# autowarefoundation/autoware_vision_pilot

Measured on AMD Instinct MI355X. Metric: frames/sec (SceneSeg+Scene3D 1280x720, one camera per GPU: preprocess + shared encoder + 2 decoder(s) + decode per frame); p50 per-frame latency beside it, higher is better.
Workload: dtype fp16x3 (hi+lo fp16 pairs on the fp16 MFMA pipe, fp32 accumulate; fp32-class: floats within 1e-3 of the fp32 oracle, 0 class flips outside that float tolerance -- tie flips only, counted per pass in profiles/r06_parity_sweep.tsv); 1 GPU; BASELINE.json metric configuration: SceneSeg+Scene3D on one 1280x720 camera per GPU, batch 1, shared EfficientNet-B0 encoder (vp_create_shared), fp16x3; precision=fp16x3, parity_mode=True, frames_in_flight_per_gpu=3, net_input=1x3x320x640, gather=False

## Files before the change

### autoware_vision_pilot_amd/csrc/engine_dispatch.cpp

```cpp
#include "engine_internal.hpp"

namespace vp {

bool Engine::plan_latency() const { return (precision_ & 32) != 0 || dev_option_is("VP_PLAN_TARGET", 'l'); }

bool plan_override(const std::string& name, int* tile, int* nsplit) {
  const char* e = dev_option("VP_PLAN_OVERRIDE");
  if (!e) return false;
  const std::string s(e);
  size_t pos = 0;
  while (pos < s.size()) {
    size_t end = s.find(';', pos);
    if (end == std::string::npos) end = s.size();
    const std::string item = s.substr(pos, end - pos);
    pos = end + 1;
    const size_t eq = item.rfind('=');
    if (eq == std::string::npos || eq == 0) continue;
    const std::string key = item.substr(0, eq), val = item.substr(eq + 1);
    if (name.size() < key.size() || name.compare(name.size() - key.size(), key.size(), key) != 0) continue;
    const size_t colon = val.find(':');
    *tile = std::atoi(val.substr(0, colon).c_str());
    *nsplit = colon == std::string::npos ? 0 : std::atoi(val.substr(colon + 1).c_str());
    return true;
  }
// ... 180 lines not shown
    if (fits && want8) halo = 8;
  }
  if ((halo == 3 || halo == 8) && q.split && q.tile < 0 && c->nsplit == 1 && q.cin_pad % 32 == 0 && !q.logits_out && !q.in2 && stride1 && plain &&
      dev_option_is("VP_X3_T16", '1') && M >= 12800)
    halo = 9;
  return halo;
}

}

ConvChoice choose_conv(const std::string& name, const ConvQuery& q) {
  const int cstride = std::max(1, q.stride);
  if (cstride > 1 && (q.ks != 3 || q.H % cstride || q.W % cstride)) throw std::invalid_argument("strided conv: 3x3 on even maps only: " + name);
  const int M = (q.H / cstride) * (q.W / cstride), ncols = round_up(q.cout, 32);
  int halo = -1, rule_nsplit = 0;
  if (q.ks == 3 && cstride == 1 && q.H >= 8 && q.W >= 16) {
    halo = base_halo_tile(q, ncols);
    halo = pipelined_tile(q, ncols, halo, &rule_nsplit);
    halo = map_tile(q, ncols, M, halo);
    if (halo == 12 && (!q.split || q.fp8_storage || !conv3x3_map2_shape_ok(q.H, q.W, q.cin_pad, round_up(ncols, 64))))
      throw std::invalid_argument("halo tile 12 (map kernel, 64-channel slabs): parity mode, maps that tile into 20x40 regions, >= 32 input channels: " + name);
    if (q.fp8_storage && q.tile < 0 && halo >= 0) halo = ncols <= 32 ? 4 : 3;
    if (halo == 11 && (q.fp8_storage || (!q.split && q.cin_pad % 32 != 0) || !conv3x3_map_shape_ok(q.H, q.W, q.cin_pad, round_up(ncols, 32))))
      throw std::invalid_argument("halo tile 11 (map kernel): maps that tile into 20x40 or 10x20 regions, >= 32 input channels (a multiple of 32 in the fp16 engines): " + name);
    if (halo >= 6 && halo <= 9 && !q.split && q.cin_pad % 64 != 0) throw std::invalid_argument("halo tiles 6 - 9 in the fp16 engines: input channels a multiple of 64: " + name);
  }
  ConvChoice c;
  if (halo >= 0) {
    const int forced = q.nsplit > 0 ? q.nsplit : rule_nsplit;
    c.bk = 32;
    c.CoutW = round_up(ncols, halo_tile_co(halo));
// ... 423 lines not shown
```

### autoware_vision_pilot_amd/csrc/kernels_conv3x3_x3.hip

```cpp
#include <algorithm>
#include <cstdlib>
#include <type_traits>

#include "conv_epilogue.hpp"
#include "lds_dma.hpp"

namespace vp {

template <int CO_TILE, int TH, int WCO, int WPX, bool HDB, int ACT, int ABL = 0, bool SPLITK = false, bool X1 = false>
__global__ __launch_bounds__(64 * WCO * WPX, (CO_TILE == 64 && TH == 8) ? 3 : 2) void conv3x3_x3_kernel(const ConvGemmParams p) {
  constexpr int NTH = 64 * WCO * WPX;
  constexpr int TW = 16, ROWB = 80, HWD = TW + 2, HPX = (TH + 2) * HWD, PX = TH * TW;
  constexpr int HALO_BYTES = HPX * ROWB, WROW = 64, W_BYTES = CO_TILE * WROW;
  constexpr int HCHUNKS = HPX * 4, HP = (HCHUNKS + NTH - 1) / NTH;
  constexpr int MT = CO_TILE / WCO / 32, NT = PX / WPX / 32;
  constexpr int NHB = HDB ? 2 : 1;
  constexpr int PL = 2;
  constexpr int HSTRIDE = HALO_BYTES;
  constexpr int LT = 0;
  constexpr int RING = HP > 3 ? HP : 3;
  static_assert(MT >= 1 && NT >= 1 && HP <= 6 && (HP <= 3 || !HDB), "tile shape");
  extern __shared__ __attribute__((aligned(16))) char smem[];
  char* const halo_base = smem;
  char* const w_base = smem + NHB * PL * HSTRIDE;
// ... 50 lines not shown
    const bool ok = hidx < HCHUNKS && (unsigned)gy < (unsigned)p.H && (unsigned)gx < (unsigned)p.W;
    h_goff[pc] = ok ? (gy * p.W + gx) * p.Cin + ch * 8 : -1;
    if constexpr ((ABL & 512) != 0) h_goff[pc] = ok ? ((gy >> 1) * (p.W >> 1) + (gx >> 1)) * p.Cin + ch * 8 : -1;
  }
  const size_t w_goff0 = (size_t)c_first * 9 * w_step + co0 * 32 + wave * 512 + lane * 8;

  f32x16_t acc[MT][NT];
#pragma unroll
  for (int i = 0; i < MT; ++i)
#pragma unroll
    for (int j = 0; j < NT; ++j)
#pragma unroll
      for (int r = 0; r < 16; ++r) acc[i][j][r] = 0.0f;

  h8_t fa[2][MT], fal[2][MT], fb[2][NT], fbl[2][NT];
  constexpr bool DIRECT_A = (ABL & 4096) != 0;
  h8_t ra[DIRECT_A ? 3 : 1][2][MT], ral[DIRECT_A ? 3 : 1][2][MT];
  const size_t w_a0 = (size_t)c_first * 9 * w_step + co0 * 32;
  u32x4 rh_hi[RING], rh_lo[RING];
#pragma unroll
  for (int r = 0; r < RING; ++r) rh_hi[r] = rh_lo[r] = zero4;
  const int s_last = KC * 9 - 1;

#define VP_DMA_W(BUF, SIDX)                                                                  \
  {                                                                                          \
    const int si_ = (SIDX) < s_last ? (SIDX) : s_last;                                       \
    const size_t base_ = (size_t)si_ * w_step + w_goff0;                                     \
    char* dst_ = w_base + (BUF) * PL * W_BYTES + wave * 1024;                                \
    _Pragma("unroll") for (int pc = 0; pc < WPIECES; ++pc) {                                 \
      VP_GLOBAL_LOAD_LDS16(p.w_hi + base_ + pc * NW * 512, dst_ + pc * NW * 1024);           \
      VP_GLOBAL_LOAD_LDS16(p.w_lo + base_ + pc * NW * 512, dst_ + W_BYTES + pc * NW * 1024); \
// ... 28 lines not shown
#define VP_READ_FRAGS(SET, WBUF, HBUF, TAPOFS)                                               \
  {                                                                                          \
    const char* wsrc_ = (WBUF) + (a_ofs0 ^ ((SET) * 32));                                    \
    if constexpr (!DIRECT_A) {                                                               \
    _Pragma("unroll") for (int i = 0; i < MT; ++i) {                                         \
      fa[SET][i] = *reinterpret_cast<const h8_t*>(wsrc_ + i * WCO * 32 * WROW);              \
      fal[SET][i] = *reinterpret_cast<const h8_t*>(wsrc_ + W_BYTES + i * WCO * 32 * WROW);   \
    }                                                                                        \
    }                                                                                        \
    _Pragma("unroll") for (int j = 0; j < NT; ++j) {                                         \
      fb[SET][j] = *reinterpret_cast<const h8_t*>((HBUF) + b_ofs0 + j * 2 * HWD * ROWB + (TAPOFS) + (SET) * 32); \
      fbl[SET][j] = *reinterpret_cast<const h8_t*>((HBUF) + HSTRIDE + b_ofs0 + j * 2 * HWD * ROWB + (TAPOFS) + (SET) * 32); \
    }                                                                                        \
  }
#define VP_MFMA(SET) VP_MFMA_RANGE(SET, 0, MT * NT)
#define VP_MFMA_RANGE(SET, Q0, Q1)                                                           \
  _Pragma("unroll") for (int q_ = (Q0); q_ < (Q1); ++q_) {                                   \
    const int i = q_ / NT, j = q_ % NT;                                                      \
    if constexpr ((ABL & 2) != 0) { acc[i][j][0] += (float)fa[SET][i][0] + (float)fal[SET][i][1] + (float)fb[SET][j][2] + (float)fbl[SET][j][3]; continue; } \
    if constexpr (DIRECT_A) {                                                                \
      acc[i][j] = __builtin_amdgcn_mfma_f32_32x32x16_f16(ral[aslot_][SET][i], fb[SET][j], acc[i][j], 0, 0, 0); \
      acc[i][j] = __builtin_amdgcn_mfma_f32_32x32x16_f16(ra[aslot_][SET][i], fbl[SET][j], acc[i][j], 0, 0, 0); \
      acc[i][j] = __builtin_amdgcn_mfma_f32_32x32x16_f16(ra[aslot_][SET][i], fb[SET][j], acc[i][j], 0, 0, 0);  \
      continue;                                                                              \
    }                                                                                        \
    if constexpr (X1) {                      \
      acc[i][j] = __builtin_amdgcn_mfma_f32_32x32x16_f16(fa[SET][i], fb[SET][j], acc[i][j], 0, 0, 0);   \
      acc[i][j] = __builtin_amdgcn_mfma_f32_32x32x16_f16(fal[SET][i], fbl[SET][j], acc[i][j], 0, 0, 0); \
      continue;                                                                              \
    }                                                                                        \
    acc[i][j] = __builtin_amdgcn_mfma_f32_32x32x16_f16(fal[SET][i], fb[SET][j], acc[i][j], 0, 0, 0); \
    acc[i][j] = __builtin_amdgcn_mfma_f32_32x32x16_f16(fa[SET][i], fbl[SET][j], acc[i][j], 0, 0, 0); \
    acc[i][j] = __builtin_amdgcn_mfma_f32_32x32x16_f16(fa[SET][i], fb[SET][j], acc[i][j], 0, 0, 0);  \
  }
#define VP_TAP(T)                                                                            \
  {                                                                                          \
    constexpr int tap_ofs_ = (((T) / 3) * HWD + ((T) % 3)) * ROWB;                           \
    constexpr int aslot_ = DIRECT_A ? (T) % 3 : 0;    \
    constexpr int tn_ = ((T) + 1) % 9;                                                       \
    constexpr int tap_next_ = ((tn_ / 3) * HWD + (tn_ % 3)) * ROWB;                          \
    const char* wcur_ = w_base + ((T) % 3) * PL * W_BYTES;                                   \
    const char* wnext_ = w_base + (((T) + 1) % 3) * PL * W_BYTES;                            \
    const char* hnext_ = ((T) == 8 && HDB) ? hbuf_other : hbuf;                              \
     \
     \
     \
     \
     \
     \
     \
     \
     \
     \
    if constexpr (HDB && (T) == 3 && !(ABL & 1) && !(ABL & 64)) {                            \
      if (next_chunk) { _Pragma("unroll") for (int pc = 0; pc < HP; ++pc) VP_STORE_H(pc, pc, hb ^ 1) } \
    }                                                                                        \
    if constexpr (DIRECT_A) {                                                                \
      if (next_chunk || (T) < 7) VP_LOAD_A(((T) + 2) % 3, c * 9 + (T) + 2)                   \
    } else if constexpr (!(ABL & 1) && !(ABL & 128)) {                                       \
      if (next_chunk || (T) < 7) VP_DMA_W(((T) + 2) % 3, c * 9 + (T) + 2)                     \
    }                                                                                        \
    __builtin_amdgcn_sched_barrier(0);                                                       \
    VP_MFMA_RANGE(0, 0, MT * NT / 2)                                                         \
    __builtin_amdgcn_sched_barrier(0);                                                       \
    if constexpr (!(ABL & 4)) VP_READ_FRAGS(1, wcur_, hbuf, tap_ofs_)                        \
    __builtin_amdgcn_sched_barrier(0);  \
    if constexpr (HDB && (T) == LT && !(ABL & 1) && !(ABL & 64)) {                           \
      _Pragma("unroll") for (int pc = 0; pc < HP; ++pc) VP_LOAD_H(pc, pc, next_chunk ? c + 1 : c) \
    }                                                                                        \
    if constexpr (!HDB && (T) < HP && !(ABL & 1) && !(ABL & 64)) {                           \
      if (next_chunk) VP_LOAD_H((T) % RING, (T) < HP ? (T) : 0, c + 1)                       \
    }                                                                                        \
    VP_MFMA_RANGE(0, MT * NT / 2, MT * NT)                                                   \
// ... 71 lines not shown
    const char* hbuf = halo_base + (HDB ? hb : 0) * PL * HSTRIDE;
    const char* hbuf_other = halo_base + (HDB ? (hb ^ 1) : 0) * PL * HSTRIDE;
    VP_TAP(0) VP_TAP(1) VP_TAP(2) VP_TAP(3) VP_TAP(4) VP_TAP(5) VP_TAP(6) VP_TAP(7) VP_TAP(8)
    hb ^= 1;
  }
  if constexpr ((ABL & 32) != 0) {
    if (blockIdx.x == 0 && tid == 0) {
      unsigned long long* dst = reinterpret_cast<unsigned long long*>(p.partial);
      dst[0] = __builtin_readcyclecounter() - probe_c0;
      dst[1] = __builtin_amdgcn_s_memrealtime() - probe_w0;
    }
  }
#undef VP_TAP
#undef VP_MFMA
#undef VP_MFMA_RANGE
#undef VP_READ_FRAGS
#undef VP_STORE_H
#undef VP_LOAD_H
#undef VP_LOAD_A
#undef VP_DMA_W

  constexpr int PITCH = CO_TILE * 2 + 16, STAGE_PLANE = PX * PITCH;
  static_assert(PL * STAGE_PLANE <= NHB * PL * HSTRIDE + 3 * PL * W_BYTES, "stage fits the main buffers");
  if constexpr ((ABL & 16) != 0) {
    if (p.H == -12345) {
#pragma unroll
      for (int i = 0; i < MT; ++i)
#pragma unroll
        for (int j = 0; j < NT; ++j)
#pragma unroll
          for (int r = 0; r < 16; ++r) p.out_f32[(i * NT + j) * 16 + r + tid * 64] = acc[i][j][r];
    }
    return;
  }
  if constexpr (SPLITK) {
    const PixPatch<TW> pixs{y0, x0, p.H, p.W};
    const int M = p.H * p.W;
#pragma unroll
// ... 53 lines not shown
    *reinterpret_cast<h8_t*>(p.out_hi + o) = *reinterpret_cast<const h8_t*>(smem + r * PITCH + c8 * 16);
    if constexpr (!X1) *reinterpret_cast<h8_t*>(p.out_lo + o) = *reinterpret_cast<const h8_t*>(smem + STAGE_PLANE + r * PITCH + c8 * 16);
  }
}

bool conv3x3_x3_supported(const ConvGemmParams& p, int shape) {
  const int co_tile = (shape == 8 || shape == 9) ? 64 : 128;
  const bool x1 = p.in_lo == nullptr;
  if (!(p.ks == 3 && p.stride <= 1 && p.in_hi && p.w_hi && p.w_lo && p.CoutW % co_tile == 0 && p.Cin % (x1 ? 64 : 32) == 0 && p.Cin2 == 0 && p.nsplit >= 1)) return false;
  const bool act_ok = x1 ? (p.act == ACT_GELU_F16 || p.act == ACT_NONE) : (p.act == ACT_GELU || p.act == ACT_NONE);
  const bool plain = p.out_hi && (x1 ? p.out_lo == nullptr : p.out_lo != nullptr) && p.store_mode == STORE_NHWC && p.res_mode == RES_NONE && p.post_act == ACT_NONE && act_ok;
  if (p.nsplit > 1) return p.partial != nullptr && p.nsplit <= p.Cin / (x1 ? 64 : 32);
  return plain;
}

template <int CO, int TH, int WPX, bool HDB, bool X1, int WCO = 2>
static hipError_t launch_x3_cfg(const ConvGemmParams& p, hipStream_t st) {
  constexpr int lds = (HDB ? 2 : 1) * 2 * ((TH + 2) * 18 * 80) + 6 * (CO * 64);
  static_assert(lds <= 160 * 1024, "LDS budget");
  constexpr int GELU = X1 ? ACT_GELU_F16 : ACT_GELU;
  const bool gelu = p.act == GELU, sk = p.nsplit > 1;
  auto k = sk ? conv3x3_x3_kernel<CO, TH, WCO, WPX, HDB, ACT_NONE, 0, true, X1>
              : (gelu ? conv3x3_x3_kernel<CO, TH, WCO, WPX, HDB, GELU, 0, false, X1> : conv3x3_x3_kernel<CO, TH, WCO, WPX, HDB, ACT_NONE, 0, false, X1>);
  static LdsAttrOnce attr_once[3];
  if (hipError_t e = set_max_dynamic_lds(attr_once[sk ? 2 : gelu], reinterpret_cast<const void*>(k), lds); e != hipSuccess) return e;
  dim3 grid(((p.H + TH - 1) / TH) * ((p.W + 15) / 16) * (p.CoutW / CO) * p.nsplit);
  hipLaunchKernelGGL(k, grid, dim3(64 * WCO * WPX), lds, st, p);
  hipError_t e = hipGetLastError();
  if (e != hipSuccess) return e;
  return sk ? launch_splitk_finish(p, st) : hipSuccess;
}

hipError_t launch_conv3x3_x3(const ConvGemmParams& p, int shape, hipStream_t st) {
  if (!conv3x3_x3_supported(p, shape)) return hipErrorInvalidValue;
  if (p.in_lo == nullptr) {
    if (shape == 6) return launch_x3_cfg<128, 16, 4, true, true>(p, st);
    if (shape == 7) return launch_x3_cfg<128, 8, 2, false, true>(p, st);
    if (shape == 8) return launch_x3_cfg<64, 8, 2, false, true>(p, st);
    if (shape == 9) return launch_x3_cfg<64, 16, 4, false, true, 1>(p, st);
    return hipErrorInvalidValue;
  }
  if (shape == 6) return launch_x3_cfg<128, 16, 4, true, false>(p, st);
  if (shape == 7) return launch_x3_cfg<128, 8, 2, false, false>(p, st);
  if (shape == 8) return launch_x3_cfg<64, 8, 2, false, false>(p, st);
  if (shape == 9) return launch_x3_cfg<64, 16, 4, false, false, 1>(p, st);
  return hipErrorInvalidValue;
}

}
```

### autoware_vision_pilot_amd/csrc/kernels_upconv.hip

```cpp
#include <algorithm>
#include <cstdlib>

#include "conv_epilogue.hpp"
#include "lds_dma.hpp"

namespace vp {

namespace {

struct PixPhase {
  int y0, x0, H, W, py, px;
  __device__ __forceinline__ int operator()(int q) const {
    int rowbit, c;
    lane_to_px16(q & 31, rowbit, c);
    const int y = y0 + 2 * (q >> 5) + rowbit, x = x0 + c;
    return (y < H && x < W) ? (2 * y + py) * (2 * W) + 2 * x + px : -1;
  }
};
struct PixRun {
  int kA, kE, W, py, px;
  __device__ __forceinline__ int operator()(int q) const {
    int rowbit, c;
    lane_to_px16(q & 31, rowbit, c);
    const int k = kA + (q >> 5) * 32 + 16 * rowbit + c;
    if (k >= kE) return -1;
    const int y = k / W, x = k - y * W;
    return (2 * y + py) * (2 * W) + 2 * x + px;
  }
};
constexpr int upconv_halo_bytes(int TH, bool CPT) { return (CPT && TH == 8) ? 192 * 80 : (TH + 2) * 18 * 80; }
constexpr int upconv_halo_capacity(int nth) { return 3 * nth / 4; }
__device__ __forceinline__ int bias_class(int m, int H2, int W2) {
  const int Y = m / W2, X = m - Y * W2;
  return (Y == 0 ? 0 : (Y == H2 - 1 ? 2 : 1)) * 3 + (X == 0 ? 0 : (X == W2 - 1 ? 2 : 1));
}

}

#define VP_WAIT_VMCNT_RT(N)                       \
  do {                                            \
    const int n_ = (N);                           \
    if (n_ >= 16) { VP_WAIT_VMCNT(16); }          \
    else if (n_ >= 14) { VP_WAIT_VMCNT(14); }     \
    else if (n_ >= 12) { VP_WAIT_VMCNT(12); }     \
    else if (n_ >= 10) { VP_WAIT_VMCNT(10); }     \
    else if (n_ >= 8) { VP_WAIT_VMCNT(8); }       \
    else if (n_ >= 6) { VP_WAIT_VMCNT(6); }       \
    else if (n_ >= 4) { VP_WAIT_VMCNT(4); }       \
    else if (n_ >= 2) { VP_WAIT_VMCNT(2); }       \
    else { VP_WAIT_VMCNT(0); }                    \
  } while (0)

template <int CO_TILE, int TH, int WCO, int WPX, bool HDB, int ACT, bool SPLITK, bool X1 = false, int ABL = 0, bool CPT = false>
__global__ __launch_bounds__(64 * WCO * WPX, 2) void upconv_x3_kernel(const UpconvParams p) {
  constexpr int NTH = 64 * WCO * WPX;
  constexpr int TW = 16, ROWB = 80, HWD = TW + 2, HPX = (TH + 2) * HWD, PX = TH * TW;
  constexpr int HALO_BYTES = upconv_halo_bytes(TH, CPT), WROW = 64, W_BYTES = CO_TILE * WROW;
  constexpr int HCHUNKS = HPX * 4, HP = (HCHUNKS + NTH - 1) / NTH;
  constexpr int MT = CO_TILE / WCO / 32, NT = PX / WPX / 32;
  constexpr int NHB = HDB ? 2 : 1;
  constexpr int PL = 2;
  constexpr int HSTRIDE = HALO_BYTES;
  static_assert(MT >= 1 && NT >= 1 && HP <= 3, "tile shape");
  extern __shared__ __attribute__((aligned(16))) char smem[];
  char* const halo_base = smem;
  char* const w_base = smem + NHB * PL * HSTRIDE;

  const int tid = threadIdx.x, lane = tid & 63, wave = tid >> 6;
// ... 91 lines not shown
    h_gs[pc] = ok ? (4 * gy * p.W + 2 * gx) * p.Cs + ch * 8 : -1;
  }
  const UpconvChunk dA = upconv_chunk(cA, py, px, CinV, CsV);
  const int S = (cB < n_chunks ? upconv_chunk(cB, py, px, CinV, CsV).step0 : upconv_steps(CinV, CsV)) - dA.step0;
  const size_t w_goff0 = ((size_t)phase * upconv_steps(CinV, CsV) + dA.step0) * w_step + co0 * 32 + wave * 512 + lane * 8;

  f32x16_t acc[MT][NT];
#pragma unroll
  for (int i = 0; i < MT; ++i)
#pragma unroll
    for (int j = 0; j < NT; ++j)
#pragma unroll
      for (int r = 0; r < 16; ++r) acc[i][j][r] = 0.0f;

  h8_t fa[2][MT], fal[2][MT], fb[2][NT], fbl[2][NT];
  u32x4 rh_hi[HP], rh_lo[HP];
#pragma unroll
  for (int r = 0; r < HP; ++r) rh_hi[r] = rh_lo[r] = zero4;

#define VP_DMA_W(WOFS, SIDX)                                                                 \
  if (!(ABL & 128) || (SIDX) < 2) {                                                          \
    const size_t base_ = (size_t)(SIDX) * w_step + w_goff0;                                  \
    char* dst_ = w_base + (WOFS) + wave * 1024;                                              \
    _Pragma("unroll") for (int pc = 0; pc < WPIECES; ++pc) {                                 \
      VP_GLOBAL_LOAD_LDS16(p.w_hi + base_ + pc * NW * 512, dst_ + pc * NW * 1024);           \
      VP_GLOBAL_LOAD_LDS16(p.w_lo + base_ + pc * NW * 512, dst_ + W_BYTES + pc * NW * 1024); \
    }                                                                                        \
  }
#define VP_LOAD_H(D)                                                                         \
  if (!(ABL & 1) || abl_prologue) {                                                          \
    const half_t* sh_ = (D).skip ? p.sk_hi : p.in_hi;                                        \
    const half_t* sl_ = (D).skip ? (VP_SK_DEAD1(D) ? p.sk_hi : sk_p1) : in_p1;               \
    const int add_ = (D).skip ? ((D).qy * 2 * p.W + (D).qx) * p.Cs + CHM * (D).ch0 : CHM * (D).ch0; \
    _Pragma("unroll") for (int pc = 0; pc < HP; ++pc) {                                      \
      const int g_ = (D).skip ? h_gs[pc] : h_gx[pc];                                         \
      const int o_ = (g_ >= 0 ? g_ + add_ : 0);                                              \
      rh_hi[pc] = *reinterpret_cast<const u32x4*>(sh_ + o_);                                 \
      rh_lo[pc] = *reinterpret_cast<const u32x4*>(sl_ + o_);                                 \
    }                                                                                        \
  }
#define VP_STORE_H(BUF, DEAD1)                                                               \
  if (!(ABL & 1) || abl_prologue)                                                            \
  _Pragma("unroll") for (int pc = 0; pc < HP; ++pc) {                                        \
    if (CPT ? h_ls[pc] >= 0 : tid + NTH * pc < HCHUNKS) {                                    \
      char* dst_ = halo_base + (BUF) * PL * HSTRIDE + (CPT ? h_ls[pc] : h_lds0 + pc * (NTH / 4) * ROWB); \
      *reinterpret_cast<u32x4*>(dst_) = h_gx[pc] >= 0 ? rh_hi[pc] : zero4;                   \
      *reinterpret_cast<u32x4*>(dst_ + HSTRIDE) = (h_gx[pc] >= 0 && !(DEAD1)) ? rh_lo[pc] : zero4; \
    }                                                                                        \
  }
#define VP_READ_FRAGS(SET, WPTR, HPTR, TAPOFS)                                               \
  {                                                                                          \
    const char* wsrc_ = (WPTR) + (a_ofs0 ^ ((SET) * 32));                                    \
    if (!CPT || nlj > 0)                                                                     \
    _Pragma("unroll") for (int i = 0; i < MT; ++i) {                                         \
      fa[SET][i] = *reinterpret_cast<const h8_t*>(wsrc_ + i * WCO * 32 * WROW);              \
      fal[SET][i] = *reinterpret_cast<const h8_t*>(wsrc_ + W_BYTES + i * WCO * 32 * WROW);   \
    }                                                                                        \
    if constexpr (CPT) {                                                                     \
      const char* hsrc_ = (HPTR) + (TAPOFS) + (SET) * 32;                                    \
      _Pragma("unroll") for (int j = 0; j < NT; ++j) {                                       \
        if (j >= nlj) continue;                                                              \
        fb[SET][j] = *reinterpret_cast<const h8_t*>(hsrc_ + b_ofs[j]);                       \
        fbl[SET][j] = *reinterpret_cast<const h8_t*>(hsrc_ + HSTRIDE + b_ofs[j]);            \
      }                                                                                      \
    } else {                                                                                 \
      const char* hsrc_ = (HPTR) + b_ofs0 + (TAPOFS) + (SET) * 32;                           \
      _Pragma("unroll") for (int j = 0; j < NT; ++j) {                                       \
        fb[SET][j] = *reinterpret_cast<const h8_t*>(hsrc_ + j * 2 * HWD * ROWB);             \
        fbl[SET][j] = *reinterpret_cast<const h8_t*>(hsrc_ + HSTRIDE + j * 2 * HWD * ROWB);  \
      }                                                                                      \
    }                                                                                        \
  }
#define VP_MFMA_RANGE(SET, Q0, Q1)                                                           \
  _Pragma("unroll") for (int q_ = (Q0); q_ < (Q1); ++q_) {                                   \
    const int i = q_ / NT, j = q_ % NT;                                                      \
    if constexpr (CPT) { if (j >= nlj) continue; }        \
    if constexpr ((ABL & 2) != 0) { acc[i][j][0] += (float)fa[SET][i][0] + (float)fal[SET][i][1] + (float)fb[SET][j][2] + (float)fbl[SET][j][3]; continue; } \
    if constexpr (X1) {                      \
      acc[i][j] = __builtin_amdgcn_mfma_f32_32x32x16_f16(fa[SET][i], fb[SET][j], acc[i][j], 0, 0, 0);   \
      acc[i][j] = __builtin_amdgcn_mfma_f32_32x32x16_f16(fal[SET][i], fbl[SET][j], acc[i][j], 0, 0, 0); \
      continue;                                                                              \
    }                                                                                        \
    acc[i][j] = __builtin_amdgcn_mfma_f32_32x32x16_f16(fal[SET][i], fb[SET][j], acc[i][j], 0, 0, 0); \
    acc[i][j] = __builtin_amdgcn_mfma_f32_32x32x16_f16(fa[SET][i], fbl[SET][j], acc[i][j], 0, 0, 0); \
    acc[i][j] = __builtin_amdgcn_mfma_f32_32x32x16_f16(fa[SET][i], fb[SET][j], acc[i][j], 0, 0, 0);  \
  }
#define VP_TAP_OFS(D, K) ((tpy + (D).a0 + ((D).nb == 2 ? ((K) >> 1) : (K))) * hrp + (tpx + (D).b0 + ((D).nb == 2 ? ((K) & 1) : 0)) * ROWB)

  bool abl_prologue = true;
  VP_LOAD_H(dA)
  VP_STORE_H(0, VP_SK_DEAD1(dA))
  VP_DMA_W(0, 0)
  if (S > 1) VP_DMA_W(PL * W_BYTES, 1)
  VP_WAIT_VMCNT(0);
  __syncthreads();
  UpconvChunk d = dA;
  UpconvChunk dn = dA;
  if (cA + 1 < cB) {
    dn = upconv_chunk(cA + 1, py, px, CinV, CsV);
    VP_LOAD_H(dn)
  }
  VP_READ_FRAGS(0, w_base, halo_base, VP_TAP_OFS(d, 0))
  abl_prologue = false;

  int c = cA, t = 0, s = 0, hb = 0;
  int w_cur = 0, w_nxt = PL * W_BYTES, w_fre = 2 * PL * W_BYTES;
#define VP_STEP(KIND, PREVLD)                                                                \
  {                                                                                          \
    const int tap_cur_ = VP_TAP_OFS(d, t);                                                   \
    const int tap_nxt_ = (KIND) == 0 ? VP_TAP_OFS(d, t + 1) : ((KIND) == 3 ? tap_cur_ : VP_TAP_OFS(dn, 0)); \
    const char* hbuf = halo_base + (HDB ? hb : 0) * PL * HSTRIDE;                            \
    const char* hbuf_next = (HDB && (KIND) != 0) ? halo_base + (hb ^ 1) * PL * HSTRIDE : hbuf; \
     \
     \
     \
    if constexpr (HDB && ((KIND) == 1 || (KIND) == 2)) { VP_STORE_H(hb ^ 1, VP_SK_DEAD1(dn)) }   \
     \
    if (s + 2 < S) VP_DMA_W(w_fre, s + 2)                                                    \
    __builtin_amdgcn_sched_barrier(0);                                                       \
    VP_MFMA_RANGE(0, 0, MT * NT / 2)                                                         \
    __builtin_amdgcn_sched_barrier(0);                                                       \
    VP_READ_FRAGS(1, w_base + w_cur, hbuf, tap_cur_)                                         \
    __builtin_amdgcn_sched_barrier(0);   \
    UpconvChunk dnn = dn;                                                                    \
    if constexpr (HDB && (KIND) == 1) {                                                      \
      dnn = upconv_chunk(c + 2, py, px, CinV, CsV);                                        \
      VP_LOAD_H(dnn)                                                                         \
    }                                                                                        \
    VP_MFMA_RANGE(0, MT * NT / 2, MT * NT)                                                   \
    __builtin_amdgcn_sched_barrier(0);                                                       \
     \
     \
    {                                                                                        \
      const int dma_n = s + 2 < S ? PL * WPIECES : 0;                                        \
      const int ld_prev = ((PREVLD) && t == 0) ? PL * HP : 0;                                \
      const int ld_this = (HDB && (KIND) == 1) ? PL * HP : 0;                                \
      VP_WAIT_VMCNT_RT(dma_n + ld_prev + ld_this);                                           \
    }                                                                                        \
     \
    VP_LDS_BARRIER();                                                                        \
    if constexpr (!HDB && ((KIND) == 1 || (KIND) == 2)) {                                    \
       \
       \
      VP_STORE_H(0, VP_SK_DEAD1(dn))                                                         \
      VP_LDS_BARRIER();                                                                      \
      if constexpr ((KIND) == 1) {                                                           \
        dnn = upconv_chunk(c + 2, py, px, CinV, CsV);                                      \
        VP_LOAD_H(dnn)                                                                       \
      }                                                                                      \
    }                                                                                        \
           \
    VP_READ_FRAGS(0, w_base + w_nxt, hbuf_next, tap_nxt_)                                    \
    __builtin_amdgcn_sched_barrier(0);                                                       \
    VP_MFMA_RANGE(1, 0, MT * NT)                                                             \
    __builtin_amdgcn_sched_barrier(0);                                                       \
                                    \
    {                                                                                        \
      const int w_old = w_cur;                                                               \
      w_cur = w_nxt;                                                                         \
      w_nxt = w_fre;                                                                         \
      w_fre = w_old;                                                                         \
    }                                                                                        \
    ++s;                                                                                     \
    if constexpr ((KIND) == 0) {                                                             \
      ++t;                                                                                   \
    } else {                                                                                 \
      ++c;                                                                                   \
      t = 0;                                                                                 \
      d = dn;                                                                                \
      dn = dnn;                                                                              \
      hb ^= 1;                                                                               \
    }                                                                                        \
  }
  while (c + 2 < cB) {
    while (t + 1 < d.nt) VP_STEP(0, true)
    VP_STEP(1, true)
  }
  if (c + 1 < cB) {
    while (t + 1 < d.nt) VP_STEP(0, true)
    VP_STEP(2, true)
  }
  while (t + 1 < d.nt) VP_STEP(0, false)
  VP_STEP(3, false)
#undef VP_STEP
#undef VP_SK_DEAD1
#undef VP_TAP_OFS
#undef VP_MFMA_RANGE
#undef VP_READ_FRAGS
#undef VP_STORE_H
#undef VP_LOAD_H
#undef VP_DMA_W

  const auto pix = [&] {
    if constexpr (CPT) return PixRun{kA, kE, p.W, py, px};
    else return PixPhase{y0, x0, p.H, p.W, py, px};
  }();
  if constexpr ((ABL & 16) != 0) {
    if (p.H == -12345) {
#pragma unroll
      for (int i = 0; i < MT; ++i)
#pragma unroll
        for (int j = 0; j < NT; ++j)
// ... 8 lines not shown
    for (int j = 0; j < NT; ++j) {
      const int m = pix((wpx * NT + j) * 32 + (lane & 31));
      if (m < 0) continue;
      float* row = p.partial + ((size_t)zsplit * M2 + m) * p.CoutW + co0 + 4 * (lane >> 5);
#pragma unroll
      for (int i = 0; i < MT; ++i)
#pragma unroll
        for (int g = 0; g < 4; ++g) {
          const f32x4_t v = {acc[i][j][4 * g + 0], acc[i][j][4 * g + 1], acc[i][j][4 * g + 2], acc[i][j][4 * g + 3]};
          *reinterpret_cast<f32x4_t*>(row + (i * WCO + wco) * 32 + 8 * g) = v;
        }
    }
    return;
  } else {
    constexpr int PITCH = CO_TILE * 2 + 16, STAGE_PLANE = PX * PITCH;
    static_assert(PL * STAGE_PLANE <= NHB * PL * HSTRIDE + 3 * PL * W_BYTES, "stage fits the main buffers");
    const float* const wsc = p.wscale + (size_t)phase * p.CoutW + co0;
    f32x4_t bb[NT][MT][4], sc[MT][4];
    int qpix[NT];
#pragma unroll
    for (int j = 0; j < NT; ++j) {
      qpix[j] = (wpx * NT + j) * 32 + (lane & 31);
      const int m = pix(qpix[j]);
      const float* const bsrc = p.bias + (size_t)(m >= 0 ? bias_class(m, 2 * p.H, 2 * p.W) : 4) * p.CoutW + co0;
#pragma unroll
      for (int i = 0; i < MT; ++i)
#pragma unroll
        for (int g = 0; g < 4; ++g) bb[j][i][g] = *reinterpret_cast<const f32x4_t*>(bsrc + (i * WCO + wco) * 32 + 4 * (lane >> 5) + 8 * g);
    }
#pragma unroll
    for (int i = 0; i < MT; ++i)
// ... 88 lines not shown
  const bool x1 = p.in_lo == nullptr;
  if (!(p.in_hi && p.w_hi && p.w_lo && p.bias && p.wscale && p.out_hi && (x1 ? p.out_lo == nullptr : p.out_lo != nullptr))) return false;
  if (p.H < 1 || p.W < 1 || p.Cin < (x1 ? 64 : 32) || p.Cin % (x1 ? 64 : 32) != 0 || p.Cs % 32 != 0 || p.Cs < 0) return false;
  if (p.Cs > 0 && !(p.sk_hi && (x1 ? p.sk_lo == nullptr : p.sk_lo != nullptr))) return false;
  if (p.CoutW % 128 != 0 || p.Ncols % 8 != 0 || p.Ncols > p.CoutW || p.Cstore < p.Ncols) return false;
  if (!(p.act == (x1 ? ACT_GELU_F16 : ACT_GELU) || p.act == ACT_NONE)) return false;
  if (p.nsplit < 1 || p.nsplit > (x1 ? upconv_chunks(p.Cin >> 1, ((p.Cs + 63) >> 6) << 5) : upconv_chunks(p.Cin, p.Cs))) return false;
  if (p.nsplit > 1 && !p.partial) return false;
  if ((long long)p.H * p.W * p.Cin >= (1ll << 31) || 4ll * p.H * p.W * std::max(p.Cs, 1) >= (1ll << 31) || 4ll * p.H * p.W * p.Cstore >= (1ll << 31)) return false;
  return true;
}

template <int TH, int WPX, bool HDB, bool X1, bool CPT = false>
static hipError_t launch_upconv_cfg(const UpconvParams& p, hipStream_t st) {
  constexpr int CO = 128;
  constexpr int lds = (HDB ? 2 : 1) * 2 * upconv_halo_bytes(TH, CPT) + 6 * (CO * 64);
  static_assert(lds <= (TH == 8 ? 80 : 160) * 1024, "LDS budget (the 4-wave shape: two workgroups per CU)");
  constexpr int GELU = X1 ? ACT_GELU_F16 : ACT_GELU;
  const bool gelu = p.act == GELU, sk = p.nsplit > 1;
  auto k = sk ? upconv_x3_kernel<CO, TH, 2, WPX, HDB, ACT_NONE, true, X1, 0, CPT>
              : (gelu ? upconv_x3_kernel<CO, TH, 2, WPX, HDB, GELU, false, X1, 0, CPT> : upconv_x3_kernel<CO, TH, 2, WPX, HDB, ACT_NONE, false, X1, 0, CPT>);
  static LdsAttrOnce attr_once[3];
  if (hipError_t e = set_max_dynamic_lds(attr_once[sk ? 2 : gelu], reinterpret_cast<const void*>(k), lds); e != hipSuccess) return e;
  const int n_px = CPT ? (p.H * p.W + TH * 16 - 1) / (TH * 16) : ((p.H + TH - 1) / TH) * ((p.W + 15) / 16);
  dim3 grid(n_px * 4 * (p.CoutW / CO) * p.nsplit);
  hipLaunchKernelGGL(k, grid, dim3(64 * 2 * WPX), lds, st, p);
  hipError_t e = hipGetLastError();
  if (e != hipSuccess || !sk) return e;
  const long long n = 4ll * p.H * p.W * (p.Ncols >> 3);
  hipLaunchKernelGGL(upconv_finish_kernel, dim3((unsigned)((n + 255) / 256)), dim3(256), 0, st, p);
  return hipGetLastError();
// ... 72 lines not shown
```

Before: 565.6 frames/s.

## Load conv weights directly into registers for the shape-7 x3 conv path

Shape 7 of the x3 3x3 conv now launches a direct-A variant whenever split-K is off. It uses 4 co-waves, one pixel wave and a double-buffered halo, and loads weight fragments from global memory straight into a 3-slot register ring instead of DMAing them into LDS. This drops the weight LDS buffers, shrinking LDS to the max of halo and staging so more workgroups fit per CU, and removes the LDS reads of weights. The upconv kernel gets the same direct-A machinery with a runtime-kind step loop, but its launcher still passes DA=false, so that path is inactive. The dispatcher also lets forced x3 tiles 106-109 apply to small maps. The risk is more register pressure and uncoalesced global weight reads per wave.

```diff
diff --git a/autoware_vision_pilot_amd/csrc/engine_dispatch.cpp b/autoware_vision_pilot_amd/csrc/engine_dispatch.cpp
--- a/autoware_vision_pilot_amd/csrc/engine_dispatch.cpp
+++ b/autoware_vision_pilot_amd/csrc/engine_dispatch.cpp
@@ -218,7 +218,8 @@
   if (cstride > 1 && (q.ks != 3 || q.H % cstride || q.W % cstride)) throw std::invalid_argument("strided conv: 3x3 on even maps only: " + name);
   const int M = (q.H / cstride) * (q.W / cstride), ncols = round_up(q.cout, 32);
   int halo = -1, rule_nsplit = 0;
-  if (q.ks == 3 && cstride == 1 && q.H >= 8 && q.W >= 16) {
+  const bool forced_x3 = q.tile >= 106 && q.tile <= 109;
+  if (q.ks == 3 && cstride == 1 && ((q.H >= 8 && q.W >= 16) || forced_x3)) {
     halo = base_halo_tile(q, ncols);
     halo = pipelined_tile(q, ncols, halo, &rule_nsplit);
     halo = map_tile(q, ncols, M, halo);
diff --git a/autoware_vision_pilot_amd/csrc/kernels_conv3x3_x3.hip b/autoware_vision_pilot_amd/csrc/kernels_conv3x3_x3.hip
--- a/autoware_vision_pilot_amd/csrc/kernels_conv3x3_x3.hip
+++ b/autoware_vision_pilot_amd/csrc/kernels_conv3x3_x3.hip
@@ -7,7 +7,12 @@
 
 namespace vp {
 
-template <int CO_TILE, int TH, int WCO, int WPX, bool HDB, int ACT, int ABL = 0, bool SPLITK = false, bool X1 = false>
+constexpr int x3_lds_bytes(int CO, int TH, bool HDB, bool DA) {
+  const int halo = (HDB ? 2 : 1) * 2 * ((TH + 2) * 18 * 80), stage = 2 * TH * 16 * (CO * 2 + 16);
+  return DA ? (halo > stage ? halo : stage) : halo + 6 * (CO * 64);
+}
+
+template <int CO_TILE, int TH, int WCO, int WPX, bool HDB, int ACT, int ABL = 0, bool SPLITK = false, bool X1 = false, bool DA = false>
 __global__ __launch_bounds__(64 * WCO * WPX, (CO_TILE == 64 && TH == 8) ? 3 : 2) void conv3x3_x3_kernel(const ConvGemmParams p) {
   constexpr int NTH = 64 * WCO * WPX;
   constexpr int TW = 16, ROWB = 80, HWD = TW + 2, HPX = (TH + 2) * HWD, PX = TH * TW;
@@ -88,7 +93,7 @@
       for (int r = 0; r < 16; ++r) acc[i][j][r] = 0.0f;
 
   h8_t fa[2][MT], fal[2][MT], fb[2][NT], fbl[2][NT];
-  constexpr bool DIRECT_A = (ABL & 4096) != 0;
+  constexpr bool DIRECT_A = DA;
   h8_t ra[DIRECT_A ? 3 : 1][2][MT], ral[DIRECT_A ? 3 : 1][2][MT];
   const size_t w_a0 = (size_t)c_first * 9 * w_step + co0 * 32;
   u32x4 rh_hi[RING], rh_lo[RING];
@@ -147,24 +152,20 @@
     }                                                                                        \
   }
 #define VP_MFMA(SET) VP_MFMA_RANGE(SET, 0, MT * NT)
+#define VP_A(SET, I) (DIRECT_A ? ra[aslot_][SET][I] : fa[SET][I])
+#define VP_AL(SET, I) (DIRECT_A ? ral[aslot_][SET][I] : fal[SET][I])
 #define VP_MFMA_RANGE(SET, Q0, Q1)                                                           \
   _Pragma("unroll") for (int q_ = (Q0); q_ < (Q1); ++q_) {                                   \
     const int i = q_ / NT, j = q_ % NT;                                                      \
-    if constexpr ((ABL & 2) != 0) { acc[i][j][0] += (float)fa[SET][i][0] + (float)fal[SET][i][1] + (float)fb[SET][j][2] + (float)fbl[SET][j][3]; continue; } \
-    if constexpr (DIRECT_A) {                                                                \
-      acc[i][j] = __builtin_amdgcn_mfma_f32_32x32x16_f16(ral[aslot_][SET][i], fb[SET][j], acc[i][j], 0, 0, 0); \
-      acc[i][j] = __builtin_amdgcn_mfma_f32_32x32x16_f16(ra[aslot_][SET][i], fbl[SET][j], acc[i][j], 0, 0, 0); \
-      acc[i][j] = __builtin_amdgcn_mfma_f32_32x32x16_f16(ra[aslot_][SET][i], fb[SET][j], acc[i][j], 0, 0, 0);  \
+    if constexpr ((ABL & 2) != 0) { acc[i][j][0] += (float)VP_A(SET, i)[0] + (float)VP_AL(SET, i)[1] + (float)fb[SET][j][2] + (float)fbl[SET][j][3]; continue; } \
+    if constexpr (X1) {                      \
+      acc[i][j] = __builtin_amdgcn_mfma_f32_32x32x16_f16(VP_A(SET, i), fb[SET][j], acc[i][j], 0, 0, 0);   \
+      acc[i][j] = __builtin_amdgcn_mfma_f32_32x32x16_f16(VP_AL(SET, i), fbl[SET][j], acc[i][j], 0, 0, 0); \
       continue;                                                                              \
     }                                                                                        \
-    if constexpr (X1) {                      \
-      acc[i][j] = __builtin_amdgcn_mfma_f32_32x32x16_f16(fa[SET][i], fb[SET][j], acc[i][j], 0, 0, 0);   \
-      acc[i][j] = __builtin_amdgcn_mfma_f32_32x32x16_f16(fal[SET][i], fbl[SET][j], acc[i][j], 0, 0, 0); \
-      continue;                                                                              \
-    }                                                                                        \
-    acc[i][j] = __builtin_amdgcn_mfma_f32_32x32x16_f16(fal[SET][i], fb[SET][j], acc[i][j], 0, 0, 0); \
-    acc[i][j] = __builtin_amdgcn_mfma_f32_32x32x16_f16(fa[SET][i], fbl[SET][j], acc[i][j], 0, 0, 0); \
-    acc[i][j] = __builtin_amdgcn_mfma_f32_32x32x16_f16(fa[SET][i], fb[SET][j], acc[i][j], 0, 0, 0);  \
+    acc[i][j] = __builtin_amdgcn_mfma_f32_32x32x16_f16(VP_AL(SET, i), fb[SET][j], acc[i][j], 0, 0, 0); \
+    acc[i][j] = __builtin_amdgcn_mfma_f32_32x32x16_f16(VP_A(SET, i), fbl[SET][j], acc[i][j], 0, 0, 0); \
+    acc[i][j] = __builtin_amdgcn_mfma_f32_32x32x16_f16(VP_A(SET, i), fb[SET][j], acc[i][j], 0, 0, 0);  \
   }
 #define VP_TAP(T)                                                                            \
   {                                                                                          \
@@ -188,8 +189,10 @@
     if constexpr (HDB && (T) == 3 && !(ABL & 1) && !(ABL & 64)) {                            \
       if (next_chunk) { _Pragma("unroll") for (int pc = 0; pc < HP; ++pc) VP_STORE_H(pc, pc, hb ^ 1) } \
     }                                                                                        \
+     \
+     \
     if constexpr (DIRECT_A) {                                                                \
-      if (next_chunk || (T) < 7) VP_LOAD_A(((T) + 2) % 3, c * 9 + (T) + 2)                   \
+      if constexpr (!(ABL & 1) && !(ABL & 128)) { if (next_chunk || (T) < 7) VP_LOAD_A(((T) + 2) % 3, c * 9 + (T) + 2) } \
     } else if constexpr (!(ABL & 1) && !(ABL & 128)) {                                       \
       if (next_chunk || (T) < 7) VP_DMA_W(((T) + 2) % 3, c * 9 + (T) + 2)                     \
     }                                                                                        \
@@ -291,6 +294,8 @@
 #undef VP_TAP
 #undef VP_MFMA
 #undef VP_MFMA_RANGE
+#undef VP_A
+#undef VP_AL
 #undef VP_READ_FRAGS
 #undef VP_STORE_H
 #undef VP_LOAD_H
@@ -298,7 +303,7 @@
 #undef VP_DMA_W
 
   constexpr int PITCH = CO_TILE * 2 + 16, STAGE_PLANE = PX * PITCH;
-  static_assert(PL * STAGE_PLANE <= NHB * PL * HSTRIDE + 3 * PL * W_BYTES, "stage fits the main buffers");
+  static_assert(PL * STAGE_PLANE <= x3_lds_bytes(CO_TILE, TH, HDB, DA), "stage fits the launch's LDS");
   if constexpr ((ABL & 16) != 0) {
     if (p.H == -12345) {
 #pragma unroll
@@ -382,14 +387,14 @@
   return plain;
 }
 
-template <int CO, int TH, int WPX, bool HDB, bool X1, int WCO = 2>
+template <int CO, int TH, int WPX, bool HDB, bool X1, int WCO = 2, bool DA = false>
 static hipError_t launch_x3_cfg(const ConvGemmParams& p, hipStream_t st) {
-  constexpr int lds = (HDB ? 2 : 1) * 2 * ((TH + 2) * 18 * 80) + 6 * (CO * 64);
-  static_assert(lds <= 160 * 1024, "LDS budget");
+  constexpr int lds = x3_lds_bytes(CO, TH, HDB, DA);
+  static_assert(lds <= (DA ? 80 : 160) * 1024, "LDS budget (direct weights: two workgroups per CU)");
   constexpr int GELU = X1 ? ACT_GELU_F16 : ACT_GELU;
   const bool gelu = p.act == GELU, sk = p.nsplit > 1;
-  auto k = sk ? conv3x3_x3_kernel<CO, TH, WCO, WPX, HDB, ACT_NONE, 0, true, X1>
-              : (gelu ? conv3x3_x3_kernel<CO, TH, WCO, WPX, HDB, GELU, 0, false, X1> : conv3x3_x3_kernel<CO, TH, WCO, WPX, HDB, ACT_NONE, 0, false, X1>);
+  auto k = sk ? conv3x3_x3_kernel<CO, TH, WCO, WPX, HDB, ACT_NONE, 0, true, X1, DA>
+              : (gelu ? conv3x3_x3_kernel<CO, TH, WCO, WPX, HDB, GELU, 0, false, X1, DA> : conv3x3_x3_kernel<CO, TH, WCO, WPX, HDB, ACT_NONE, 0, false, X1, DA>);
   static LdsAttrOnce attr_once[3];
   if (hipError_t e = set_max_dynamic_lds(attr_once[sk ? 2 : gelu], reinterpret_cast<const void*>(k), lds); e != hipSuccess) return e;
   dim3 grid(((p.H + TH - 1) / TH) * ((p.W + 15) / 16) * (p.CoutW / CO) * p.nsplit);
@@ -409,7 +414,7 @@
     return hipErrorInvalidValue;
   }
   if (shape == 6) return launch_x3_cfg<128, 16, 4, true, false>(p, st);
-  if (shape == 7) return launch_x3_cfg<128, 8, 2, false, false>(p, st);
+  if (shape == 7) return p.nsplit > 1 ? launch_x3_cfg<128, 8, 2, false, false>(p, st) : launch_x3_cfg<128, 8, 1, true, false, 4, true>(p, st);
   if (shape == 8) return launch_x3_cfg<64, 8, 2, false, false>(p, st);
   if (shape == 9) return launch_x3_cfg<64, 16, 4, false, false, 1>(p, st);
   return hipErrorInvalidValue;
diff --git a/autoware_vision_pilot_amd/csrc/kernels_upconv.hip b/autoware_vision_pilot_amd/csrc/kernels_upconv.hip
--- a/autoware_vision_pilot_amd/csrc/kernels_upconv.hip
+++ b/autoware_vision_pilot_amd/csrc/kernels_upconv.hip
@@ -29,6 +29,10 @@
   }
 };
 constexpr int upconv_halo_bytes(int TH, bool CPT) { return (CPT && TH == 8) ? 192 * 80 : (TH + 2) * 18 * 80; }
+constexpr int upconv_lds_bytes(int TH, bool HDB, bool CPT, bool DA) {
+  const int halo = (HDB ? 2 : 1) * 2 * upconv_halo_bytes(TH, CPT), stage = 2 * TH * 16 * (128 * 2 + 16);
+  return DA ? (halo > stage ? halo : stage) : halo + 6 * (128 * 64);
+}
 constexpr int upconv_halo_capacity(int nth) { return 3 * nth / 4; }
 __device__ __forceinline__ int bias_class(int m, int H2, int W2) {
   const int Y = m / W2, X = m - Y * W2;
@@ -51,7 +55,7 @@
     else { VP_WAIT_VMCNT(0); }                    \
   } while (0)
 
-template <int CO_TILE, int TH, int WCO, int WPX, bool HDB, int ACT, bool SPLITK, bool X1 = false, int ABL = 0, bool CPT = false>
+template <int CO_TILE, int TH, int WCO, int WPX, bool HDB, int ACT, bool SPLITK, bool X1 = false, int ABL = 0, bool CPT = false, bool DA = false>
 __global__ __launch_bounds__(64 * WCO * WPX, 2) void upconv_x3_kernel(const UpconvParams p) {
   constexpr int NTH = 64 * WCO * WPX;
   constexpr int TW = 16, ROWB = 80, HWD = TW + 2, HPX = (TH + 2) * HWD, PX = TH * TW;
@@ -173,6 +177,8 @@
       for (int r = 0; r < 16; ++r) acc[i][j][r] = 0.0f;
 
   h8_t fa[2][MT], fal[2][MT], fb[2][NT], fbl[2][NT];
+  h8_t ra[DA ? 3 : 1][2][MT], ral[DA ? 3 : 1][2][MT];
+  const size_t w_a0 = ((size_t)phase * upconv_steps(CinV, CsV) + dA.step0) * w_step + co0 * 32;
   u32x4 rh_hi[HP], rh_lo[HP];
 #pragma unroll
   for (int r = 0; r < HP; ++r) rh_hi[r] = rh_lo[r] = zero4;
@@ -184,6 +190,17 @@
     _Pragma("unroll") for (int pc = 0; pc < WPIECES; ++pc) {                                 \
       VP_GLOBAL_LOAD_LDS16(p.w_hi + base_ + pc * NW * 512, dst_ + pc * NW * 1024);           \
       VP_GLOBAL_LOAD_LDS16(p.w_lo + base_ + pc * NW * 512, dst_ + W_BYTES + pc * NW * 1024); \
+    }                                                                                        \
+  }
+#define VP_LOAD_A(RSLOT, SIDX)                                                               \
+  if (!(ABL & 128) || abl_prologue) {                                                        \
+    const int si_ = (SIDX) < S - 1 ? (SIDX) : S - 1;                                         \
+    const size_t base_ = (size_t)si_ * w_step + w_a0;                                        \
+    _Pragma("unroll") for (int ss_ = 0; ss_ < 2; ++ss_)                                      \
+    _Pragma("unroll") for (int i = 0; i < MT; ++i) {                                         \
+      const size_t o_ = base_ + (size_t)(((a_ofs0 ^ (ss_ * 32)) + i * WCO * 32 * WROW) >> 1); \
+      ra[RSLOT][ss_][i] = *reinterpret_cast<const h8_t*>(p.w_hi + o_);                       \
+      ral[RSLOT][ss_][i] = *reinterpret_cast<const h8_t*>(p.w_lo + o_);                      \
     }                                                                                        \
   }
 #define VP_LOAD_H(D)                                                                         \
@@ -210,7 +227,7 @@
 #define VP_READ_FRAGS(SET, WPTR, HPTR, TAPOFS)                                               \
   {                                                                                          \
     const char* wsrc_ = (WPTR) + (a_ofs0 ^ ((SET) * 32));                                    \
-    if (!CPT || nlj > 0)                                                                     \
+    if (!DA && (!CPT || nlj > 0))                                                            \
     _Pragma("unroll") for (int i = 0; i < MT; ++i) {                                         \
       fa[SET][i] = *reinterpret_cast<const h8_t*>(wsrc_ + i * WCO * 32 * WROW);              \
       fal[SET][i] = *reinterpret_cast<const h8_t*>(wsrc_ + W_BYTES + i * WCO * 32 * WROW);   \
@@ -230,27 +247,34 @@
       }                                                                                      \
     }                                                                                        \
   }
+#define VP_A(SET, I) (DA ? ra[aslot_][SET][I] : fa[SET][I])
+#define VP_AL(SET, I) (DA ? ral[aslot_][SET][I] : fal[SET][I])
 #define VP_MFMA_RANGE(SET, Q0, Q1)                                                           \
   _Pragma("unroll") for (int q_ = (Q0); q_ < (Q1); ++q_) {                                   \
     const int i = q_ / NT, j = q_ % NT;                                                      \
     if constexpr (CPT) { if (j >= nlj) continue; }        \
-    if constexpr ((ABL & 2) != 0) { acc[i][j][0] += (float)fa[SET][i][0] + (float)fal[SET][i][1] + (float)fb[SET][j][2] + (float)fbl[SET][j][3]; continue; } \
+    if constexpr ((ABL & 2) != 0) { acc[i][j][0] += (float)VP_A(SET, i)[0] + (float)VP_AL(SET, i)[1] + (float)fb[SET][j][2] + (float)fbl[SET][j][3]; continue; } \
     if constexpr (X1) {                      \
-      acc[i][j] = __builtin_amdgcn_mfma_f32_32x32x16_f16(fa[SET][i], fb[SET][j], acc[i][j], 0, 0, 0);   \
-      acc[i][j] = __builtin_amdgcn_mfma_f32_32x32x16_f16(fal[SET][i], fbl[SET][j], acc[i][j], 0, 0, 0); \
+      acc[i][j] = __builtin_amdgcn_mfma_f32_32x32x16_f16(VP_A(SET, i), fb[SET][j], acc[i][j], 0, 0, 0);   \
+      acc[i][j] = __builtin_amdgcn_mfma_f32_32x32x16_f16(VP_AL(SET, i), fbl[SET][j], acc[i][j], 0, 0, 0); \
       continue;                                                                              \
     }                                                                                        \
-    acc[i][j] = __builtin_amdgcn_mfma_f32_32x32x16_f16(fal[SET][i], fb[SET][j], acc[i][j], 0, 0, 0); \
-    acc[i][j] = __builtin_amdgcn_mfma_f32_32x32x16_f16(fa[SET][i], fbl[SET][j], acc[i][j], 0, 0, 0); \
-    acc[i][j] = __builtin_amdgcn_mfma_f32_32x32x16_f16(fa[SET][i], fb[SET][j], acc[i][j], 0, 0, 0);  \
+    acc[i][j] = __builtin_amdgcn_mfma_f32_32x32x16_f16(VP_AL(SET, i), fb[SET][j], acc[i][j], 0, 0, 0); \
+    acc[i][j] = __builtin_amdgcn_mfma_f32_32x32x16_f16(VP_A(SET, i), fbl[SET][j], acc[i][j], 0, 0, 0); \
+    acc[i][j] = __builtin_amdgcn_mfma_f32_32x32x16_f16(VP_A(SET, i), fb[SET][j], acc[i][j], 0, 0, 0);  \
   }
 #define VP_TAP_OFS(D, K) ((tpy + (D).a0 + ((D).nb == 2 ? ((K) >> 1) : (K))) * hrp + (tpx + (D).b0 + ((D).nb == 2 ? ((K) & 1) : 0)) * ROWB)
 
   bool abl_prologue = true;
   VP_LOAD_H(dA)
   VP_STORE_H(0, VP_SK_DEAD1(dA))
-  VP_DMA_W(0, 0)
-  if (S > 1) VP_DMA_W(PL * W_BYTES, 1)
+  if constexpr (DA) {
+    VP_LOAD_A(0, 0)
+    VP_LOAD_A(1, 1)
+  } else {
+    VP_DMA_W(0, 0)
+    if (S > 1) VP_DMA_W(PL * W_BYTES, 1)
+  }
   VP_WAIT_VMCNT(0);
   __syncthreads();
   UpconvChunk d = dA;
@@ -264,25 +288,35 @@
 
   int c = cA, t = 0, s = 0, hb = 0;
   int w_cur = 0, w_nxt = PL * W_BYTES, w_fre = 2 * PL * W_BYTES;
-#define VP_STEP(KIND, PREVLD)                                                                \
+#define VP_STEP(KIND, PREVLD, R)                                                             \
   {                                                                                          \
+    constexpr int aslot_ = (R);                                                              \
+    constexpr bool rt_ = (KIND) < 0;                                                         \
+    const bool k_last_ = rt_ ? t + 1 >= d.nt : (KIND) != 0;                                  \
+    const bool k_store_ = rt_ ? (k_last_ && c + 1 < cB) : ((KIND) == 1 || (KIND) == 2);      \
+    const bool k_refill_ = rt_ ? (k_last_ && c + 2 < cB) : (KIND) == 1;                      \
+    const bool k_end_ = rt_ ? (k_last_ && c + 1 >= cB) : (KIND) == 3;                        \
     const int tap_cur_ = VP_TAP_OFS(d, t);                                                   \
-    const int tap_nxt_ = (KIND) == 0 ? VP_TAP_OFS(d, t + 1) : ((KIND) == 3 ? tap_cur_ : VP_TAP_OFS(dn, 0)); \
+    const int tap_nxt_ = !k_last_ ? VP_TAP_OFS(d, t + 1) : (k_end_ ? tap_cur_ : VP_TAP_OFS(dn, 0)); \
     const char* hbuf = halo_base + (HDB ? hb : 0) * PL * HSTRIDE;                            \
-    const char* hbuf_next = (HDB && (KIND) != 0) ? halo_base + (hb ^ 1) * PL * HSTRIDE : hbuf; \
-     \
-     \
-     \
-    if constexpr (HDB && ((KIND) == 1 || (KIND) == 2)) { VP_STORE_H(hb ^ 1, VP_SK_DEAD1(dn)) }   \
-     \
-    if (s + 2 < S) VP_DMA_W(w_fre, s + 2)                                                    \
+    const char* hbuf_next = (HDB && k_last_) ? halo_base + (hb ^ 1) * PL * HSTRIDE : hbuf;   \
+     \
+     \
+     \
+    if (HDB && k_store_) { VP_STORE_H(hb ^ 1, VP_SK_DEAD1(dn)) }                             \
+     \
+     \
+     \
+     \
+    if constexpr (DA) { VP_LOAD_A(((R) + 2) % 3, s + 2) }                                    \
+    else if (s + 2 < S) VP_DMA_W(w_fre, s + 2)                                               \
     __builtin_amdgcn_sched_barrier(0);                                                       \
     VP_MFMA_RANGE(0, 0, MT * NT / 2)                                                         \
     __builtin_amdgcn_sched_barrier(0);                                                       \
     VP_READ_FRAGS(1, w_base + w_cur, hbuf, tap_cur_)                                         \
     __builtin_amdgcn_sched_barrier(0);   \
     UpconvChunk dnn = dn;                                                                    \
-    if constexpr (HDB && (KIND) == 1) {                                                      \
+    if (HDB && k_refill_) {                                                                  \
       dnn = upconv_chunk(c + 2, py, px, CinV, CsV);                                        \
       VP_LOAD_H(dnn)                                                                         \
     }                                                                                        \
@@ -290,20 +324,20 @@
     __builtin_amdgcn_sched_barrier(0);                                                       \
      \
      \
-    {                                                                                        \
+    if constexpr (!DA) {               \
       const int dma_n = s + 2 < S ? PL * WPIECES : 0;                                        \
       const int ld_prev = ((PREVLD) && t == 0) ? PL * HP : 0;                                \
-      const int ld_this = (HDB && (KIND) == 1) ? PL * HP : 0;                                \
+      const int ld_this = (HDB && k_refill_) ? PL * HP : 0;                                  \
       VP_WAIT_VMCNT_RT(dma_n + ld_prev + ld_this);                                           \
     }                                                                                        \
      \
     VP_LDS_BARRIER();                                                                        \
-    if constexpr (!HDB && ((KIND) == 1 || (KIND) == 2)) {                                    \
+    if (!HDB && k_store_) {                                                                  \
        \
        \
       VP_STORE_H(0, VP_SK_DEAD1(dn))                                                         \
       VP_LDS_BARRIER();                                                                      \
-      if constexpr ((KIND) == 1) {                                                           \
+      if (k_refill_) {                                                                       \
         dnn = upconv_chunk(c + 2, py, px, CinV, CsV);                                      \
         VP_LOAD_H(dnn)                                                                       \
       }                                                                                      \
@@ -321,7 +355,7 @@
       w_fre = w_old;                                                                         \
     }                                                                                        \
     ++s;                                                                                     \
-    if constexpr ((KIND) == 0) {                                                             \
+    if (!k_last_) {                                                                          \
       ++t;                                                                                   \
     } else {                                                                                 \
       ++c;                                                                                   \
@@ -331,20 +365,34 @@
       hb ^= 1;                                                                               \
     }                                                                                        \
   }
-  while (c + 2 < cB) {
-    while (t + 1 < d.nt) VP_STEP(0, true)
-    VP_STEP(1, true)
-  }
-  if (c + 1 < cB) {
-    while (t + 1 < d.nt) VP_STEP(0, true)
-    VP_STEP(2, true)
-  }
-  while (t + 1 < d.nt) VP_STEP(0, false)
-  VP_STEP(3, false)
+  if constexpr (DA) {
+    for (;;) {
+      VP_STEP(-1, true, 0)
+      if (s >= S) break;
+      VP_STEP(-1, true, 1)
+      if (s >= S) break;
+      VP_STEP(-1, true, 2)
+      if (s >= S) break;
+    }
+  } else {
+    while (c + 2 < cB) {
+      while (t + 1 < d.nt) VP_STEP(0, true, 0)
+      VP_STEP(1, true, 0)
+    }
+    if (c + 1 < cB) {
+      while (t + 1 < d.nt) VP_STEP(0, true, 0)
+      VP_STEP(2, true, 0)
+    }
+    while (t + 1 < d.nt) VP_STEP(0, false, 0)
+    VP_STEP(3, false, 0)
+  }
 #undef VP_STEP
 #undef VP_SK_DEAD1
 #undef VP_TAP_OFS
 #undef VP_MFMA_RANGE
+#undef VP_A
+#undef VP_AL
+#undef VP_LOAD_A
 #undef VP_READ_FRAGS
 #undef VP_STORE_H
 #undef VP_LOAD_H
@@ -383,7 +431,7 @@
     return;
   } else {
     constexpr int PITCH = CO_TILE * 2 + 16, STAGE_PLANE = PX * PITCH;
-    static_assert(PL * STAGE_PLANE <= NHB * PL * HSTRIDE + 3 * PL * W_BYTES, "stage fits the main buffers");
+    static_assert(PL * STAGE_PLANE <= upconv_lds_bytes(TH, HDB, CPT, DA), "stage fits the launch's LDS");
     const float* const wsc = p.wscale + (size_t)phase * p.CoutW + co0;
     f32x4_t bb[NT][MT][4], sc[MT][4];
     int qpix[NT];
@@ -502,7 +550,7 @@
 template <int TH, int WPX, bool HDB, bool X1, bool CPT = false>
 static hipError_t launch_upconv_cfg(const UpconvParams& p, hipStream_t st) {
   constexpr int CO = 128;
-  constexpr int lds = (HDB ? 2 : 1) * 2 * upconv_halo_bytes(TH, CPT) + 6 * (CO * 64);
+  constexpr int lds = upconv_lds_bytes(TH, HDB, CPT, false);
   static_assert(lds <= (TH == 8 ? 80 : 160) * 1024, "LDS budget (the 4-wave shape: two workgroups per CU)");
   constexpr int GELU = X1 ? ACT_GELU_F16 : ACT_GELU;
   const bool gelu = p.act == GELU, sk = p.nsplit > 1;
```

Result: no change. 568.9 frames/s, median of 6 (+0.6%).
